# macoustics/ap-vast-unofficial

Hardware: AMD Instinct MI355X
Metric: subband filter-updates/sec (blocks x bins / s), 16-spk/32-mic/1024-bin (higher is better)
Workload: dtype f64

## Files before the change

ap_vast_unofficial_amd/csrc/gevd16_common.h:

```cpp
#pragma once
#include <type_traits>
#include "apv_internal.h"

namespace {

constexpr int N = 16;
constexpr int LD = 17;

template <typename T> struct Cx { T x, y; };
template <typename T> __device__ __forceinline__ Cx<T> mk(T a, T b) { Cx<T> r; r.x = a; r.y = b; return r; }

template <typename T> struct Prec;
template <> struct Prec<double> {
    static constexpr double sweep_tol2 = 1e-16;
    static constexpr int max_sweeps = 14;
};
template <> struct Prec<float> {
    static constexpr float sweep_tol2 = 1e-8f;
    static constexpr int max_sweeps = 12;
};

__device__ __forceinline__ double rsq_full(double x) {
    double y = __builtin_amdgcn_rsq(x);
    const double t = x * y;
    const double e = __builtin_fma(-t, y, 1.0);
    const double pp = __builtin_fma(0.375, e, 0.5);
    const double ye = y * e;
    return __builtin_fma(ye, pp, y);
}
__device__ __forceinline__ double rcp_full(double x) {
    double y = __builtin_amdgcn_rcp(x);
    y = y * __builtin_fma(-x, y, 2.0);
    return y * __builtin_fma(-x, y, 2.0);
}
__device__ __forceinline__ float rcp_full(float x) {
    const float y = __builtin_amdgcn_rcpf(x);
    return y * __builtin_fmaf(-x, y, 2.0f);
}
__device__ __forceinline__ float rsq_full(float x) {
    float y = __builtin_amdgcn_rsqf(x);
    const float t = x * y;
    const float e = __builtin_fmaf(-t, y, 1.0f);
    return __builtin_fmaf(y * e, 0.5f, y);
}

__device__ __forceinline__ void wsync() { __syncthreads(); }

template <typename T> __device__ __forceinline__ T wave_sum(T v) {
#pragma unroll
    for (int o = 32; o >= 1; o >>= 1) v += __shfl_xor(v, o, 64);
    return __shfl(v, 0, 64);
}

__device__ __forceinline__ float uniform_scalar(float v) { return __int_as_float(__builtin_amdgcn_readfirstlane(__float_as_int(v))); }
__device__ __forceinline__ double uniform_scalar(double v) {
    return __hiloint2double(__builtin_amdgcn_readfirstlane(__double2hiint(v)), __builtin_amdgcn_readfirstlane(__double2loint(v)));
}

using d4 = __attribute__((ext_vector_type(4))) double;
using f4 = __attribute__((ext_vector_type(4))) float;

template <typename T> struct Mfma16;
__device__ __forceinline__ float fma_t(float a, float b, float c) { return __builtin_fmaf(a, b, c); }
__device__ __forceinline__ double fma_t(double a, double b, double c) { return __builtin_fma(a, b, c); }

template <> struct Mfma16<double> {
    using V = d4;
    static __device__ __forceinline__ V mac(double a, double b, V c) { return __builtin_amdgcn_mfma_f64_16x16x4f64(a, b, c, 0, 0, 0); }
    static __device__ __forceinline__ int row(int lane, int t) { return (lane >> 4) + 4 * t; }
};
template <> struct Mfma16<float> {
    using V = f4;
    static __device__ __forceinline__ V mac(float a, float b, V c) { return __builtin_amdgcn_mfma_f32_16x16x4f32(a, b, c, 0, 0, 0); }
    static __device__ __forceinline__ int row(int lane, int t) { return 4 * (lane >> 4) + t; }
};

struct NoStamp { __device__ __forceinline__ void operator()(int) const {} };
template <typename T, typename XT, bool WITH_D, typename ST = NoStamp, int GS = 1>
__device__ __forceinline__ void correlate16(const XT* __restrict__ X, const XT* __restrict__ dvec, int M,
                                            Cx<T>* dst, Cx<T>* sr, int lane, ST stamp = ST(), int stamp_base = 0) {
    using MM = Mfma16<T>;
    typename MM::V re = {0, 0, 0, 0}, im = {0, 0, 0, 0};
    T rx = 0, ry = 0;
    const int msub = lane >> 4;
    XT zero;
    zero.x = 0;
    zero.y = 0;
    auto chunk = [&](int mc, auto full_tag) {
        constexpr bool FULL = decltype(full_tag)::value;
        XT xv[8], dv[8];
        const XT* const xrow0 = X + ((size_t)(mc + msub) * N + (lane & 15)) * GS;
        const XT* const drow0 = WITH_D ? dvec + mc + msub : nullptr;
#pragma unroll
        for (int q = 0; q < 8; ++q) {
            const int m = mc + 4 * q + msub;
            const bool ok = FULL || m < M;
            XT xl, dl = zero;
            if constexpr (FULL) {
                xl = xrow0[(size_t)(4 * q) * N * GS];
                if constexpr (WITH_D) dl = drow0[4 * q];
            } else {
                const int mcl = ok ? m : M - 1;
                xl = X[((size_t)mcl * N + (lane & 15)) * GS];
                if constexpr (WITH_D) dl = dvec[mcl];
            }
            xv[q].x = ok ? xl.x : zero.x;
            xv[q].y = ok ? xl.y : zero.y;
            dv[q].x = ok ? dl.x : zero.x;
            dv[q].y = ok ? dl.y : zero.y;
        }
        if constexpr (!__is_same(ST, NoStamp)) {
            asm volatile("s_waitcnt vmcnt(0)" ::: "memory");
            stamp(stamp_base);
        }
#pragma unroll
        for (int q = 0; q < 8; ++q) {
            const T xr = (T)xv[q].x, xi = (T)xv[q].y;
            re = MM::mac(xr, xr, re);
            re = MM::mac(xi, xi, re);
            im = MM::mac(xr, xi, im);
            if constexpr (WITH_D) {
                rx = fma_t(xi, (T)dv[q].y, fma_t(xr, (T)dv[q].x, rx));
                ry = fma_t(-xi, (T)dv[q].x, fma_t(xr, (T)dv[q].y, ry));
            }
        }
    };
    if ((M & 31) == 0) {
        for (int mc = 0; mc < M; mc += 32) chunk(mc, std::true_type{});
    } else {
        for (int mc = 0; mc < M; mc += 32) chunk(mc, std::false_type{});
    }
    const int col = lane & 15;
#pragma unroll
    for (int t = 0; t < 4; ++t) dst[MM::row(lane, t) * LD + col] = mk<T>(re[t], im[t]);
    stamp(stamp_base + 1);
    wsync();
    T pt[4];
#pragma unroll
    for (int t = 0; t < 4; ++t) pt[t] = dst[col * LD + MM::row(lane, t)].y;
    wsync();
#pragma unroll
    for (int t = 0; t < 4; ++t) dst[MM::row(lane, t) * LD + col].y = im[t] - pt[t];
    if constexpr (WITH_D) {
        rx += __shfl_xor(rx, 16, 64); ry += __shfl_xor(ry, 16, 64);
        rx += __shfl_xor(rx, 32, 64); ry += __shfl_xor(ry, 32, 64);
        if (lane < N) sr[lane] = mk<T>(rx, ry);
    }
}



struct XStep { signed char tbit, delta; };
constexpr XStep XSCHED[2][15] = {
    {{-1, 1}, {-1, 2}, {-1, 1}, {-1, 4}, {-1, 1}, {-1, 2}, {-1, 1}, {-1, 4}, {2, 1}, {-1, 2}, {-1, 1}, {-1, 2}, {1, 1}, {-1, 1}, {0, 0}},
    {{-1, 1}, {-1, 2}, {-1, 1}, {-1, 4}, {-1, 1}, {-1, 2}, {-1, 1}, {-1, 4}, {0, 2}, {-1, 4}, {-1, 2}, {-1, 4}, {1, 4}, {-1, 4}, {2, 0}}};
constexpr unsigned long long xs_pack(int sweep, bool tb) {
    unsigned long long v = 0;
    for (int r = 0; r < 15; ++r)
        v |= (unsigned long long)(tb ? (XSCHED[sweep][r].tbit + 1) : XSCHED[sweep][r].delta) << (4 * r);
    return v;
}
constexpr unsigned long long XS_DELTA0 = xs_pack(0, false), XS_DELTA1 = xs_pack(1, false);
constexpr unsigned long long XS_TBIT0 = xs_pack(0, true), XS_TBIT1 = xs_pack(1, true);

template <typename T> __device__ __forceinline__ Cx<T> cshfl(Cx<T> v, int src) {
    return mk<T>(__shfl(v.x, src, 64), __shfl(v.y, src, 64));
}
template <typename T> __device__ __forceinline__ void xchg(Cx<T>& top, Cx<T>& bot, bool bit, int peer) {
    const Cx<T> send = bit ? top : bot;
    const Cx<T> recv = cshfl(send, peer);
    if (bit) top = recv; else bot = recv;
}

template <int D> __device__ __forceinline__ int dpp_xor_lo(int v);
template <> __device__ __forceinline__ int dpp_xor_lo<1>(int v) { return __builtin_amdgcn_mov_dpp(v, 0xB1, 0xf, 0xf, false); }
template <> __device__ __forceinline__ int dpp_xor_lo<2>(int v) { return __builtin_amdgcn_mov_dpp(v, 0x4E, 0xf, 0xf, false); }
template <> __device__ __forceinline__ int dpp_xor_lo<4>(int v) { return __builtin_amdgcn_ds_swizzle(v, 0x101F); }
__device__ __forceinline__ int dpp_xor8(int v) { return __builtin_amdgcn_mov_dpp(v, 0x128, 0xf, 0xf, false); }

template <int D> __device__ __forceinline__ float xcol(float v) { return __int_as_float(dpp_xor_lo<D>(__float_as_int(v))); }
template <int D> __device__ __forceinline__ double xcol(double v) {
    return __hiloint2double(dpp_xor_lo<D>(__double2hiint(v)), dpp_xor_lo<D>(__double2loint(v)));
}
template <int D> __device__ __forceinline__ float xrow(float v, int lane) {
    if constexpr (D == 1) return __int_as_float(dpp_xor8(__float_as_int(v)));
    else return __int_as_float(__builtin_amdgcn_ds_bpermute((lane ^ (8 * D)) << 2, __float_as_int(v)));
}
template <int D> __device__ __forceinline__ double xrow(double v, int lane) {
    if constexpr (D == 1) return __hiloint2double(dpp_xor8(__double2hiint(v)), dpp_xor8(__double2loint(v)));
    else {
        const int addr = (lane ^ (8 * D)) << 2;
        return __hiloint2double(__builtin_amdgcn_ds_bpermute(addr, __double2hiint(v)),
                                __builtin_amdgcn_ds_bpermute(addr, __double2loint(v)));
    }
}
template <int TB> __device__ __forceinline__ void xswap_row(int& top, int& bot) {
    if constexpr (TB == 0) {
        const int nt = __builtin_amdgcn_update_dpp(top, bot, 0x128, 0xf, 0xc, false);
        bot = __builtin_amdgcn_update_dpp(bot, top, 0x128, 0xf, 0x3, false);
        top = nt;
    } else if constexpr (TB == 1) {
        const auto r = __builtin_amdgcn_permlane16_swap((unsigned)top, (unsigned)bot, false, false);
        top = (int)r[0];
        bot = (int)r[1];
    } else {
        const auto r = __builtin_amdgcn_permlane32_swap((unsigned)top, (unsigned)bot, false, false);
        top = (int)r[0];
        bot = (int)r[1];
    }
}
__device__ __forceinline__ void xswap_col4(int& top, int& bot) {
    const int nt = __builtin_amdgcn_update_dpp(top, bot, 0x114, 0xf, 0xa, false);
    bot = __builtin_amdgcn_update_dpp(bot, top, 0x104, 0xf, 0x5, false);
    top = nt;
}
template <int TB> __device__ __forceinline__ void xswap_row(float& t, float& b) {
    int ti = __float_as_int(t), bi = __float_as_int(b);
    xswap_row<TB>(ti, bi);
    t = __int_as_float(ti);
    b = __int_as_float(bi);
}
template <int TB> __device__ __forceinline__ void xswap_row(double& t, double& b) {
    int tl = __double2loint(t), th = __double2hiint(t), bl = __double2loint(b), bh = __double2hiint(b);
    xswap_row<TB>(tl, bl);
    xswap_row<TB>(th, bh);
    t = __hiloint2double(th, tl);
    b = __hiloint2double(bh, bl);
}
__device__ __forceinline__ void xswap_col4(float& t, float& b) {
    int ti = __float_as_int(t), bi = __float_as_int(b);
    xswap_col4(ti, bi);
    t = __int_as_float(ti);
    b = __int_as_float(bi);
}
__device__ __forceinline__ void xswap_col4(double& t, double& b) {
    int tl = __double2loint(t), th = __double2hiint(t), bl = __double2loint(b), bh = __double2hiint(b);
    xswap_col4(tl, bl);
    xswap_col4(th, bh);
    t = __hiloint2double(th, tl);
    b = __hiloint2double(bh, bl);
}
template <int TB, typename T> __device__ __forceinline__ void cxswap_row(Cx<T>& t, Cx<T>& b) {
    xswap_row<TB>(t.x, b.x);
    xswap_row<TB>(t.y, b.y);
}
template <typename T> __device__ __forceinline__ void cxswap_col4(Cx<T>& t, Cx<T>& b) {
    xswap_col4(t.x, b.x);
    xswap_col4(t.y, b.y);
}

template <int D, typename T> __device__ __forceinline__ Cx<T> cxcol(Cx<T> v) { return mk<T>(xcol<D>(v.x), xcol<D>(v.y)); }
template <int D, typename T> __device__ __forceinline__ Cx<T> cxrow(Cx<T> v, int lane) { return mk<T>(xrow<D>(v.x, lane), xrow<D>(v.y, lane)); }

template <int D, typename T>
__device__ __forceinline__ void move_bottoms(Cx<T>& tb, Cx<T>& bt, Cx<T>& bb, Cx<T>& v0b, Cx<T>& v1b, int lane) {
    tb = cxcol<D>(tb);
    v0b = cxcol<D>(v0b);
    v1b = cxcol<D>(v1b);
    bb = cxcol<D>(bb);
    bt = cxrow<D>(bt, lane);
    bb = cxrow<D>(bb, lane);
}

template <typename T>
__device__ __forceinline__ void rot_cols(T c, Cx<T> s, Cx<T> p, Cx<T> q, Cx<T>& po, Cx<T>& qo) {
    po.x = c * p.x - (s.x * q.x + s.y * q.y);
    po.y = c * p.y - (s.x * q.y - s.y * q.x);
    qo.x = c * q.x + (s.x * p.x - s.y * p.y);
    qo.y = c * q.y + (s.x * p.y + s.y * p.x);
}
template <typename T>
__device__ __forceinline__ void rot_rows(T c, Cx<T> s, Cx<T> p, Cx<T> q, Cx<T>& po, Cx<T>& qo) {
    po.x = c * p.x - (s.x * q.x - s.y * q.y);
    po.y = c * p.y - (s.x * q.y + s.y * q.x);
    qo.x = c * q.x + (s.x * p.x + s.y * p.y);
    qo.y = c * q.y + (s.x * p.y - s.y * p.x);
}
using f2v = __attribute__((ext_vector_type(2))) float;
using f4v = __attribute__((ext_vector_type(4))) float;
__device__ __forceinline__ f2v pk_cmul(f2v s, f2v z) {
    const f2v t = {-s.y, s.y};
    return __builtin_elementwise_fma((f2v){s.x, s.x}, z, t * (f2v){z.y, z.x});
}
__device__ __forceinline__ f2v pk_cmulc(f2v s, f2v z) {
    const f2v t = {s.y, -s.y};
    return __builtin_elementwise_fma((f2v){s.x, s.x}, z, t * (f2v){z.y, z.x});
}
template <>
__device__ __forceinline__ void rot_cols<float>(float c, Cx<float> s, Cx<float> p, Cx<float> q, Cx<float>& po, Cx<float>& qo) {
    const f2v cc = {c, c}, sv = {s.x, s.y}, pv = {p.x, p.y}, qv = {q.x, q.y};
    const f2v a = cc * pv - pk_cmulc(sv, qv), b = cc * qv + pk_cmul(sv, pv);
    po = mk<float>(a.x, a.y);
    qo = mk<float>(b.x, b.y);
}
template <>
__device__ __forceinline__ void rot_rows<float>(float c, Cx<float> s, Cx<float> p, Cx<float> q, Cx<float>& po, Cx<float>& qo) {
    const f2v cc = {c, c}, sv = {s.x, s.y}, pv = {p.x, p.y}, qv = {q.x, q.y};
    const f2v a = cc * pv - pk_cmul(sv, qv), b = cc * qv + pk_cmulc(sv, pv);
    po = mk<float>(a.x, a.y);
    qo = mk<float>(b.x, b.y);
}

template <typename T>
__device__ __forceinline__ void rotation(T alpha, T gamma, T bx, T by, T& c, T& sx, T& sy) {
    const float fbx = (float)bx, fby = (float)by, fd = (float)(gamma - alpha);
    const float b2 = fbx * fbx + fby * fby;
    if constexpr (sizeof(T) == 4) {
        const float zeta = 0.5f * fd;
        const float x = fmaxf(__builtin_fmaf(zeta, zeta, b2), 1e-36f);
        const float hh = x * __builtin_amdgcn_rsqf(x);
        const float D = fmaxf(fabsf(zeta), 1e-18f) + hh;
        const float rr = __builtin_amdgcn_rsqf((hh + hh) * D);
        const float rs = copysignf(rr, zeta);
        c = D * rr;
        sx = fbx * rs;
        sy = fby * rs;
        return;
    }
    float tx = 0.f, ty = 0.f;
    if (b2 > 1e-30f) {
        const float iab = __builtin_amdgcn_rsqf(b2);
        const float tau = fd * 0.5f * iab;
        const float rho = __builtin_amdgcn_sqrtf(__builtin_fmaf(tau, tau, 1.0f));
        const float t = copysignf(__builtin_amdgcn_rcpf(fabsf(tau) + rho), tau) * iab;
        tx = fbx * t;
        ty = fby * t;
    }
    const T dx = (T)tx, dy = (T)ty;
    c = rsq_full((T)1 + dx * dx + dy * dy);
    sx = dx * c;
    sy = dy * c;
}

template <typename TT>
__device__ __forceinline__ int jacobi16_sweeps(Cx<TT>& tt_, Cx<TT>& tb_, Cx<TT>& bt_, Cx<TT>& bb_, Cx<TT>& v0t_, Cx<TT>& v0b_,
                                               Cx<TT>& v1t_, Cx<TT>& v1b_, TT (*srot)[4], int lane, TT tol2, TT normS2,
                                               int max_sweeps, bool& converged_, int n_rounds = 15) {
    using CC = Cx<TT>;
    const int a = lane >> 3, b = lane & 7;
    const bool diag = (a == b);
    int sweeps_done = 0;
    bool converged = false;
    CC tt = tt_, tb = tb_, bt = bt_, bb = bb_, v0t = v0t_, v0b = v0b_, v1t = v1t_, v1b = v1b_;
    for (int sweep = 0; sweep < max_sweeps && !converged; ++sweep) {
        TT off = 0;
        const unsigned long long dseq = (sweep & 1) ? XS_DELTA1 : XS_DELTA0;
        const unsigned long long tseq = (sweep & 1) ? XS_TBIT1 : XS_TBIT0;
        for (int r = 0; r < n_rounds; ++r) {
            const int delta = (int)((dseq >> (4 * r)) & 15), tbit = (int)((tseq >> (4 * r)) & 15) - 1;
            if (tbit >= 0) {
                if (tbit == 2) {
                    cxswap_col4(tt, tb);
                    cxswap_col4(bt, bb);
                    cxswap_col4(v0t, v0b);
                    cxswap_col4(v1t, v1b);
                    cxswap_row<2>(tt, bt);
                    cxswap_row<2>(tb, bb);
                } else {
                    const bool cb_ = (b >> tbit) & 1;
                    const int pc = lane ^ (1 << tbit);
                    xchg(tt, tb, cb_, pc);
                    xchg(bt, bb, cb_, pc);
                    xchg(v0t, v0b, cb_, pc);
                    xchg(v1t, v1b, cb_, pc);
                    if (tbit == 1) {
                        cxswap_row<1>(tt, bt);
                        cxswap_row<1>(tb, bb);
                    } else {
                        cxswap_row<0>(tt, bt);
                        cxswap_row<0>(tb, bb);
                    }
                }
            }
            switch (delta) {
                case 1: move_bottoms<1>(tb, bt, bb, v0b, v1b, lane); break;
                case 2: move_bottoms<2>(tb, bt, bb, v0b, v1b, lane); break;
                case 4: move_bottoms<4>(tb, bt, bb, v0b, v1b, lane); break;
                default: break;
            }
            if (diag) off += tb.x * tb.x + tb.y * tb.y;
            TT c, sx, sy;
            rotation<TT>(tt.x, bb.x, tb.x, tb.y, c, sx, sy);
            TT ca, sax, say, cb, sbx, sby;
            if constexpr (sizeof(TT) == 8) {
                if (diag) {
                    srot[a][0] = c;
                    srot[a][1] = sx;
                    srot[a][2] = sy;
                }
                wsync();
                ca = srot[a][0]; sax = srot[a][1]; say = srot[a][2];
                cb = srot[b][0]; sbx = srot[b][1]; sby = srot[b][2];
            } else {
                const int da = 9 * a, db = 9 * b;
                ca = __shfl(c, da, 64); sax = __shfl(sx, da, 64); say = __shfl(sy, da, 64);
                cb = __shfl(c, db, 64); sbx = __shfl(sx, db, 64); sby = __shfl(sy, db, 64);
            }
            const CC sa = mk<TT>(sax, say), sb = mk<TT>(sbx, sby);
            CC ypp, ypq, yqp, yqq;
            rot_cols<TT>(cb, sb, tt, tb, ypp, ypq);
            rot_cols<TT>(cb, sb, bt, bb, yqp, yqq);
            rot_rows<TT>(ca, sa, ypp, yqp, tt, bt);
            rot_rows<TT>(ca, sa, ypq, yqq, tb, bb);
            if (diag) {
                tt.y = 0;
                bb.y = 0;
            }
            CC w0p, w0q, w1p, w1q;
            rot_cols<TT>(cb, sb, v0t, v0b, w0p, w0q);
            rot_cols<TT>(cb, sb, v1t, v1b, w1p, w1q);
            v0t = w0p; v0b = w0q; v1t = w1p; v1b = w1q;
        }
// ... 316 lines not shown
```

ap_vast_unofficial_amd/csrc/kernels_gevd16m.hip:

```cpp
#include "apv_internal.h"

#include <cstdlib>

#include "gevd16_common.h"

namespace {

__device__ __forceinline__ float tp_lane(float v, int l) { return __int_as_float(__builtin_amdgcn_readlane(__float_as_int(v), l)); }
__device__ __forceinline__ float tp_from(float v, int src) { return __int_as_float(__builtin_amdgcn_ds_bpermute(src << 2, __float_as_int(v))); }
__device__ __forceinline__ float tp_quad_bcast(float v, int j) {
    const int x = __float_as_int(v);
    return __int_as_float(j == 0 ? __builtin_amdgcn_mov_dpp(x, 0x00, 0xf, 0xf, false) : j == 1 ? __builtin_amdgcn_mov_dpp(x, 0x55, 0xf, 0xf, false)
                          : j == 2 ? __builtin_amdgcn_mov_dpp(x, 0xAA, 0xf, 0xf, false) : __builtin_amdgcn_mov_dpp(x, 0xFF, 0xf, 0xf, false));
}
template <int CTRL> __device__ __forceinline__ void tp_dpp_add(float& v) {
    v += __int_as_float(__builtin_amdgcn_update_dpp(0, __float_as_int(v), CTRL, 0xf, 0xf, true));
    asm volatile("" : "+v"(v));
}
__device__ __forceinline__ float tp_sum_quad(float v) { tp_dpp_add<0xB1>(v); tp_dpp_add<0x4E>(v); return v; }
__device__ __forceinline__ float tp_sum_quads(float v) {
    tp_dpp_add<0x128>(v);
    tp_dpp_add<0x124>(v);
    asm("s_nop 1\n\tv_add_f32_dpp %0, %0, %0 row_bcast:15 row_mask:0xa bank_mask:0xf\n\t"
        "s_nop 1\n\tv_add_f32_dpp %0, %0, %0 row_bcast:31 row_mask:0xc bank_mask:0xf" : "+v"(v));
// ... 337 lines not shown
        }
        const T inv2 = rcp_full(dkk);
        const C li2 = mk<T>(li.x * inv2, li.y * inv2);
#pragma unroll
        for (int t = 0; t < 4; ++t) {
            if (4 * t + 3 <= kk) continue;
            brow[t].x = fma_t(-li2.y, lj[t].y, fma_t(-li2.x, lj[t].x, brow[t].x));
            brow[t].y = fma_t(li2.x, lj[t].y, fma_t(-li2.y, lj[t].x, brow[t].y));
        }
        if (i > kk) {
#pragma unroll
            for (int t = 0; t < 4; ++t) {
                if (4 * t > kk) continue;
                wrow[t].x = fma_t(li2.y, wk[t].y, fma_t(-li2.x, wk[t].x, wrow[t].x));
                wrow[t].y = fma_t(-li2.y, wk[t].x, fma_t(-li2.x, wk[t].y, wrow[t].y));
            }
        }
    }
    wsync();
    {
        const T di = ccol[i][i].x;
        if (__any(!(di > (T)0) || !(di < (T)3.0e38))) status = 1;
        if (status == 0) {
            const T ri = rsq_full(di);
#pragma unroll
            for (int t = 0; t < 4; ++t) wrow[t] = mk<T>(wrow[t].x * ri, wrow[t].y * ri);
        }
    }
    stamp(2);
    if (dstop == 2) return;

    if (status == 0) {
#pragma unroll
        for (int t = 0; t < 4; ++t) sB[i * LD + jq + 4 * t] = wrow[t];
        wsync();
        C acc[4];
        const int col = lane & 15;
        cmm16([&](int r, int kx) { return sB[r * LD + kx]; }, [&](int kx, int c) { return sA[kx * LD + c]; }, lane, acc);
        wsync();
#pragma unroll
        for (int t = 0; t < 4; ++t) sA[mfma_row<T>(lane, t) * LD + col] = acc[t];
        wsync();
        cmm16([&](int r, int kx) { return sA[r * LD + kx]; },
              [&](int kx, int c) { const C w = sB[c * LD + kx]; return mk<T>(w.x, -w.y); }, lane, acc);
        wsync();
        T nrm = 0;
#pragma unroll
        for (int t = 0; t < 4; ++t) {
            const int row = mfma_row<T>(lane, t);
            if (row == col) acc[t].y = 0;
            sA[row * LD + col] = acc[t];
            nrm += acc[t].x * acc[t].x + acc[t].y * acc[t].y;
        }
        const T normF2 = uniform_scalar(wave_sum(nrm));
        wsync();
        stamp(3);
        if (dstop == 3) return;

        const int a = lane >> 3, b = lane & 7;
        const int max_sweeps = p.max_sweeps > 0 ? p.max_sweeps : Prec<T>::max_sweeps;
        const T tol2 = p.sweep_tol2 > 0.0 ? (T)p.sweep_tol2 : Prec<T>::sweep_tol2;
        bool converged = false;
        const int sexp = __builtin_amdgcn_readfirstlane((normF2 > (T)0) ? -((sizeof(T) == 8 ? ilogb((double)normF2) : ilogbf((float)normF2)) / 2) : 0);
        T normS2;
        if constexpr (sizeof(T) == 8) normS2 = uniform_scalar((T)ldexp((double)normF2, 2 * sexp));
        else normS2 = uniform_scalar((T)ldexpf((float)normF2, 2 * sexp));
        bool v_in_lds = false, refined = false;
        auto spectrum_ok = [&](float nt, float nb) {
            float mn = fminf(nt, nb), mx = fmaxf(nt, nb);
#pragma unroll
            for (int m = 1; m < 64; m <<= 1) {
                mn = fminf(mn, __shfl_xor(mn, m, 64));
                mx = fmaxf(mx, __shfl_xor(mx, m, 64));
            }
            return !__any(!(mn >= 1e-3f * mx));
        };
        if constexpr (sizeof(T) == 8) {
            if (dstop != 4) {
                using CF = Cx<float>;
                CF v32[4];
                CF* const fQ = reinterpret_cast<CF*>(&sB[0]);
                const bool trust = tridiag_presolve16<T>(sA, sexp, (float)normS2, fQ, reinterpret_cast<float*>(fQ + N * LDQ), lane, v32, stamp);
                if (!trust) {
                    wsync();
#pragma unroll
                    for (int t = 0; t < 4; ++t) sB[i * LD + jq + 4 * t] = wrow[t];
                    wsync();
                } else {
                const int mcol = lane & 15;
                auto cj = [](C w) { return mk<T>(w.x, -w.y); };
                wsync();
#pragma unroll
                for (int t = 0; t < 4; ++t) sB[mfma_row<float>(lane, t) * LD + mcol] = mk<T>((T)v32[t].x, (T)v32[t].y);
                wsync();
                C accT[4], accG[4], accC[4], accV[4];
                cmm16([&](int r, int kx) { return sA[r * LD + kx]; }, [&](int kx, int c) { return sB[kx * LD + c]; }, lane, accT);
                cmm16([&](int r, int kx) { return cj(sB[kx * LD + r]); }, [&](int kx, int c) { return sB[kx * LD + c]; }, lane, accG);
                wsync();
#pragma unroll
                for (int t = 0; t < 4; ++t) sA[mfma_row<T>(lane, t) * LD + mcol] = accT[t];
                wsync();
                cmm16([&](int r, int kx) { return cj(sB[kx * LD + r]); }, [&](int kx, int c) { return sA[kx * LD + c]; }, lane, accC);
                constexpr double kRefineGuard2 = 9e-10;
                constexpr double kSecondStep2 = 1e-4;
                const bool refine_ok = (dstop != 5) && !(p.sweep_tol2 > 0.0);
                T* const sLam2 = reinterpret_cast<T*>(&scoef[0]);
                for (int step = 0; step < 2; ++step) {
                    {
                        T num = (T)0, gd = (T)1;
                        bool has_diag = false;
#pragma unroll
                        for (int t = 0; t < 4; ++t) {
                            const bool d = mfma_row<T>(lane, t) == mcol;
                            num = d ? accC[t].x : num;
                            gd = d ? accG[t].x : gd;
                            has_diag = has_diag || d;
                        }
                        T ginv = __builtin_amdgcn_rcp(gd);
                        ginv = ginv * __builtin_fma(-gd, ginv, (T)2);
                        T quot = num * ginv;
                        quot = __builtin_fma(__builtin_fma(-gd, quot, num), ginv, quot);
                        if (has_diag) sLam[mcol] = quot;
                    }
                    wsync();
                    bool bad = false, hopeless = false;
                    const T dj = sLam[mcol];
                    T l2 = (T)0;
#pragma unroll
                    for (int t = 0; t < 4; ++t) {
                        const int row = mfma_row<T>(lane, t);
                        const T di = sLam[row];
                        C z;
                        if (row == mcol) {
                            z = mk<T>((T)0.5 * ((T)1 - accG[t].x), (T)0);
                        } else {
                            const T den = dj - di;
                            T inv = __builtin_amdgcn_rcp(den);
                            inv = inv * __builtin_fma(-den, inv, (T)2);
                            const T zx = __builtin_fma(-dj, accG[t].x, accC[t].x) * inv, zy = __builtin_fma(-dj, accG[t].y, accC[t].y) * inv;
                            const T zz = zx * zx + zy * zy;
                            bad = bad || !(zz <= (T)kRefineGuard2);
                            hopeless = hopeless || !(zz <= (T)kSecondStep2);
                            z = mk<T>(zx, zy);
                            l2 = __builtin_fma(zz, den, l2);
                        }
                        sA[row * LD + mcol] = z;
                    }
                    l2 += __shfl_xor(l2, 16, 64);
                    l2 += __shfl_xor(l2, 32, 64);
                    if (lane < N) sLam2[mcol] = l2 + dj;
                    const bool pass = !__any(bad) || dstop == 10;
                    if (dstop == 9 && !pass) status = 8 << step;
                    if (!refine_ok || (!pass && (step == 1 || __any(hopeless)))) break;
                    wsync();
                    auto v_step = [&]() {
                        cmm16([&](int r, int kx) { return sB[r * LD + kx]; }, [&](int kx, int c) { return sA[kx * LD + c]; }, lane, accV);
#pragma unroll
                        for (int t = 0; t < 4; ++t) {
                            const C v = sB[mfma_row<T>(lane, t) * LD + mcol];
                            accV[t] = mk<T>(v.x + accV[t].x, v.y + accV[t].y);
                        }
                    };
                    if (pass) {
                        v_step();
                        if (lane < N) sLam[lane] = sLam2[lane];
                        wsync();
#pragma unroll
                        for (int t = 0; t < 4; ++t) {
                            sA[mfma_row<T>(lane, t) * LD + mcol] = accV[t];
                            sB[i * LD + jq + 4 * t] = wrow[t];
                        }
                        wsync();
                        refined = true;
                        break;
                    }
                    if constexpr (sizeof(T) == 8) {
                        auto ipz = [&](int r, int c) { const C zv = sA[r * LD + c]; return mk<T>(zv.x + (r == c ? (T)1 : (T)0), zv.y); };
                        cmm16x([&](int s_, int, int) { return cj(accC[s_]); }, [&](int, int kx, int c) { return ipz(kx, c); }, lane, accT);
                        cmm16x([&](int, int r, int kx) { return cj(ipz(kx, r)); }, [&](int s_, int, int) { return accT[s_]; }, lane, accC);
#pragma unroll
                        for (int t = 0; t < 4; ++t)
                            if (mfma_row<T>(lane, t) == mcol) accC[t].y = 0;
                        v_step();
                        wsync();
#pragma unroll
                        for (int t = 0; t < 4; ++t) sB[mfma_row<T>(lane, t) * LD + mcol] = accV[t];
                        wsync();
                        cmm16([&](int r, int kx) { return cj(sB[kx * LD + r]); }, [&](int kx, int c) { return sB[kx * LD + c]; }, lane, accG);
                    }
                }
                if (!refined) {
                    constexpr int n_it = 4;
                    {
                    for (int it = 0; it < n_it; ++it) {
                        wsync();
#pragma unroll
                        for (int t = 0; t < 4; ++t) {
                            const int row = mfma_row<T>(lane, t);
                            sA[row * LD + mcol] = mk<T>((row == mcol ? (T)1.5 : (T)0) - (T)0.5 * accG[t].x, (T)-0.5 * accG[t].y);
                        }
                        wsync();
                        cmm16([&](int r, int kx) { return sB[r * LD + kx]; }, [&](int kx, int c) { return sA[kx * LD + c]; }, lane, accV);
                        cmm16x([&](int s_, int, int) { return cj(accC[s_]); }, [&](int, int kx, int c) { return sA[kx * LD + c]; }, lane, accT);
                        cmm16x([&](int, int r, int kx) { return sA[r * LD + kx]; }, [&](int s_, int, int) { return accT[s_]; }, lane, accC);
                        wsync();
#pragma unroll
                        for (int t = 0; t < 4; ++t) {
                            sB[mfma_row<T>(lane, t) * LD + mcol] = accV[t];
                            if (mfma_row<T>(lane, t) == mcol) accC[t].y = 0;
                        }
                        wsync();
                        if (it + 1 < n_it)
                            cmm16([&](int r, int kx) { return cj(sB[kx * LD + r]); }, [&](int kx, int c) { return sB[kx * LD + c]; }, lane, accG);
                    }
#pragma unroll
                    for (int t = 0; t < 4; ++t) sA[mfma_row<T>(lane, t) * LD + mcol] = accC[t];
                    wsync();
                    }
                    v_in_lds = true;
                }
                }
            }
        }
        if constexpr (sizeof(T) == 4) {
            constexpr int LDF = 17;
            constexpr float kShift = 8e-6f;
            const float delta = kShift * sqrtf((float)normS2);
            Cx<float>* const fG = reinterpret_cast<Cx<float>*>(&sB[0]);
            Cx<float> (*const fcol)[16] = reinterpret_cast<Cx<float>(*)[16]>(&scol[0][0]);
            chol16_f32<T, LD, LDF>(sA, sexp, delta, fG, fcol, lane);
            const int oa = lane & 7, ob = lane >> 3;
            Cx<float> g0t = fG[(2 * oa) * LDF + ob], g0b = fG[(2 * oa) * LDF + 8 + ob];
            Cx<float> g1t = fG[(2 * oa + 1) * LDF + ob], g1b = fG[(2 * oa + 1) * LDF + 8 + ob];
            float n2t, n2b;
            (void)jacobi16_onesided<LDF>(g0t, g0b, g1t, g1b, lane, (float)tol2, (float)normS2, max_sweeps, converged, n2t, n2b, fG);
            const bool trust = converged && spectrum_ok(n2t, n2b);
            converged = false;
            wsync();
#pragma unroll
            for (int t = 0; t < 4; ++t) sB[i * LD + jq + 4 * t] = wrow[t];
            if (trust) {
                const int it_b = os_top_end(ob), ib_b = os_bot_end(ob);
                wsync();
                sA[(2 * oa) * LD + it_b] = mk<T>(g0t.x, g0t.y);
                sA[(2 * oa) * LD + ib_b] = mk<T>(g0b.x, g0b.y);
                sA[(2 * oa + 1) * LD + it_b] = mk<T>(g1t.x, g1t.y);
                sA[(2 * oa + 1) * LD + ib_b] = mk<T>(g1b.x, g1b.y);
                if (oa == 0) {
                    sLam[it_b] = (T)ldexpf(n2t - delta, -sexp);
                    sLam[ib_b] = (T)ldexpf(n2b - delta, -sexp);
                }
                refined = true;
            }
            wsync();
        }
        if (!refined) {
            C tt = sA[a * LD + b], tb = sA[a * LD + 8 + b], bt = sA[(8 + a) * LD + b], bb = sA[(8 + a) * LD + 8 + b];
            const T scl = (sizeof(T) == 8) ? (T)ldexp(1.0, sexp) : (T)ldexpf(1.0f, sexp);
            tt = mk<T>(tt.x * scl, tt.y * scl); tb = mk<T>(tb.x * scl, tb.y * scl);
            bt = mk<T>(bt.x * scl, bt.y * scl); bb = mk<T>(bb.x * scl, bb.y * scl);
            C v0t = mk<T>((2 * a == b) ? (T)1 : (T)0, 0), v0b = mk<T>((2 * a == 8 + b) ? (T)1 : (T)0, 0);
            C v1t = mk<T>((2 * a + 1 == b) ? (T)1 : (T)0, 0), v1b = mk<T>((2 * a + 1 == 8 + b) ? (T)1 : (T)0, 0);
            if (v_in_lds) {
                v0t = sB[(2 * a) * LD + b]; v0b = sB[(2 * a) * LD + 8 + b];
                v1t = sB[(2 * a + 1) * LD + b]; v1b = sB[(2 * a + 1) * LD + 8 + b];
                wsync();
    #pragma unroll
                for (int t = 0; t < 4; ++t) sB[i * LD + jq + 4 * t] = wrow[t];
            }
            const bool diag = (a == b);
            const int sweeps_done = jacobi16_sweeps<T>(tt, tb, bt, bb, v0t, v0b, v1t, v1b, srot, lane, tol2, normS2, max_sweeps, converged);
            if (!converged) status = 2;
            const bool nat = sweeps_done & 1;
            const int it_b = nat ? 2 * b : b, ib_b = nat ? 2 * b + 1 : 8 + b;
            wsync();
            sA[(2 * a) * LD + it_b] = v0t;
            sA[(2 * a) * LD + ib_b] = v0b;
            sA[(2 * a + 1) * LD + it_b] = v1t;
            sA[(2 * a + 1) * LD + ib_b] = v1b;
            if (diag) {
                const T iscl = (sizeof(T) == 8) ? (T)ldexp(1.0, -sexp) : (T)ldexpf(1.0f, -sexp);
                sLam[it_b] = tt.x * iscl;
                sLam[ib_b] = bb.x * iscl;
            }
            wsync();
        }

        stamp(6);
        {
            const int i16 = lane & 15, q4 = lane >> 4;
            const T li = sLam[i16];
            int rank = 0;
#pragma unroll
            for (int jj = 0; jj < 4; ++jj) {
                const int j = 4 * q4 + jj;
                const T lj = sLam[j];
                rank += (lj > li) || (lj == li && j < i16);
            }
            rank += __shfl_xor(rank, 16, 64);
            rank += __shfl_xor(rank, 32, 64);
            if (q4 == 0) sOrder[rank] = i16;
        }

        cmm16([&](int r, int kx) { const C w = sB[kx * LD + r]; return mk<T>(w.x, -w.y); },
              [&](int kx, int c) { return sA[kx * LD + c]; }, lane, acc);
        wsync();
#pragma unroll
        for (int t = 0; t < 4; ++t) sA[mfma_row<T>(lane, t) * LD + col] = acc[t];
        wsync();

        {
            const int i16 = lane & 15, q4 = lane >> 4;
            T sx = 0, sy = 0;
#pragma unroll
            for (int ll = 0; ll < 4; ++ll) {
                const int l = 4 * q4 + ll;
                const C v = sA[l * LD + i16], rr = sr[l];
                sx = fma_t(v.y, rr.y, fma_t(v.x, rr.x, sx));
                sy = fma_t(-v.y, rr.x, fma_t(v.x, rr.y, sy));
            }
            sx += __shfl_xor(sx, 16, 64); sy += __shfl_xor(sy, 16, 64);
            sx += __shfl_xor(sx, 32, 64); sy += __shfl_xor(sy, 32, 64);
            if (q4 == 0) {
                const T den = rcp_full(sLam[i16] + span_mu<true, T>(p.span, z1, k, p.mu));
                scoef[i16] = mk<T>(sx * den, sy * den);
            }
        }
        wsync();
    }

    {
        const int i16 = lane & 15;
        T ax = 0, ay = 0;
        int done = lane >> 4;
        const int s_k = span_limit<true, T>(p.span, z1, k, N, p.ranks[p.nV - 1], status != 1, !HOPS || hop == p.span.last_hop, sLam,
                                      scoef, sOrder, lane);
        for (int t = 0; t < p.nV; ++t) {
            const int V = min(p.ranks[t], s_k);
            if (status != 1) {
                for (; done < V; done += 4) {
                    const int c = sOrder[done];
                    const C cf = scoef[c], v = sA[i16 * LD + c];
                    ax = fma_t(-cf.y, v.y, fma_t(cf.x, v.x, ax));
                    ay = fma_t(cf.y, v.x, fma_t(cf.x, v.y, ay));
                }
            }
            T wx = ax + __shfl_xor(ax, 16, 64), wy = ay + __shfl_xor(ay, 16, 64);
            wx += __shfl_xor(wx, 32, 64); wy += __shfl_xor(wy, 32, 64);
            if (lane < N) {
                const size_t o = ((size_t)k * p.nV + t) * N + lane;
                if (p.out_c128) reinterpret_cast<double2*>(pw)[o] = make_double2((double)wx, (double)wy);
                else reinterpret_cast<float2*>(pw)[o] = make_float2((float)wx, (float)wy);
            }
        }
    }
    if (lane < N) {
        if (plam != nullptr) {
            const T lv = (status != 1) ? sLam[sOrder[lane]] : (T)0;
            if (p.out_c128) reinterpret_cast<double*>(plam)[(size_t)k * N + lane] = (double)lv;
            else reinterpret_cast<float*>(plam)[(size_t)k * N + lane] = (float)lv;
        }
    }
    if (p.U != nullptr) {
        C* U = reinterpret_cast<C*>(p.U) + (size_t)k * N * N;
#pragma unroll
        for (int t = 0; t < 4; ++t) {
            const int idx = lane + 64 * t, ii = idx >> 4, j = idx & 15;
            U[idx] = (status != 1) ? sA[ii * LD + sOrder[j]] : mk<T>(0, 0);
        }
    }
    if (pstatus != nullptr && lane == 0) pstatus[k] = status;
    stamp(7);
}

template <typename T, bool FUSED, typename XT, bool DBG = false>
__global__ void __launch_bounds__(64) gevd16m_kernel(const GevdParams p) { gevd16m_body<T, FUSED, XT, DBG>(p, blockIdx.x, blockIdx.y == 1); }
template <bool FUSED, typename XT, bool DBG = false>
__global__ void __launch_bounds__(64) __attribute__((amdgpu_waves_per_eu(4, 4))) gevd16m_kernel_f64(const GevdParams p) {
    gevd16m_body<double, FUSED, XT, DBG>(p, blockIdx.x, blockIdx.y == 1);
}
template <int GS>
__global__ void __launch_bounds__(64) __attribute__((amdgpu_waves_per_eu(4, 4))) gevd16m_kernel_f64_grouped(const GevdParams p) {
    constexpr int BLK = 8 * GS;
    const int id = blockIdx.x;
    const int k = ((id | (BLK - 1)) < p.K) ? ((id & ~(BLK - 1)) | ((id & 7) * GS) | ((id >> 3) & (GS - 1))) : id;
    gevd16m_body<double, true, double2, false, GS>(p, k, blockIdx.y == 1);
}
template <int GS>
__global__ void __launch_bounds__(64) __attribute__((amdgpu_waves_per_eu(4, 4))) gevd16m_kernel_f64_hops(const GevdParams p) {
    constexpr int BLK = 8 * GS;
    const int id = blockIdx.x;
    const int k = (GS > 1 && (id | (BLK - 1)) < p.K) ? ((id & ~(BLK - 1)) | ((id & 7) * GS) | ((id >> 3) & (GS - 1))) : id;
    gevd16m_body<double, true, double2, false, GS, true>(p, k, blockIdx.y == 1, blockIdx.z);
}

__global__ void __launch_bounds__(64) __attribute__((amdgpu_waves_per_eu(4, 4))) gevd16m_kernel_f64_hops_c64(const GevdParams p) {
    gevd16m_body<double, true, float2, false, 1, true>(p, blockIdx.x, blockIdx.y == 1, blockIdx.z);
}
__global__ void __launch_bounds__(64) gevd16m_kernel_f32_hops_c64(const GevdParams p) {
    gevd16m_body<float, true, float2, false, 1, true>(p, blockIdx.x, blockIdx.y == 1, blockIdx.z);
}

}

bool apv_gevd16m_takes_hops(const GevdParams& p, int compute_dtype, bool fused) {
    if (!(p.n == 16 && p.reg_mode == APV_REG_ABS && p.reg_bright == 0.0 && fused && p.debug_stop == 0 && p.stamps == nullptr && p.n_hops <= 65535))
        return false;
    if (p.x_c128) return compute_dtype == APV_F64 && (p.x_group <= 1 || p.x_group == 4);
    return p.x_group <= 1;
}

hipError_t apv_launch_gevd16m(const GevdParams& p, int compute_dtype, bool fused, hipStream_t s) {
    if (p.n != 16 || p.reg_mode != APV_REG_ABS || p.reg_bright != 0.0) return hipErrorNotSupported;
    if (p.K <= 0) return hipSuccess;
    const dim3 grid(p.K, p.n_zones > 1 ? 2 : 1);
    const bool xd = fused && p.x_c128;
    if (p.n_hops > 1) {
        if (!apv_gevd16m_takes_hops(p, compute_dtype, fused)) return hipErrorInvalidValue;
        const dim3 grid3(p.K, p.n_zones > 1 ? 2 : 1, p.n_hops);
        if (!p.x_c128) {
            if (compute_dtype == APV_F64) hipLaunchKernelGGL(gevd16m_kernel_f64_hops_c64, grid3, dim3(64), 0, s, p);
            else hipLaunchKernelGGL(gevd16m_kernel_f32_hops_c64, grid3, dim3(64), 0, s, p);
            return hipGetLastError();
        }
        if (p.x_group == 4) hipLaunchKernelGGL(gevd16m_kernel_f64_hops<4>, grid3, dim3(64), 0, s, p);
        else hipLaunchKernelGGL(gevd16m_kernel_f64_hops<1>, grid3, dim3(64), 0, s, p);
        return hipGetLastError();
    }
    if (p.x_group > 1) {
        if (!xd || compute_dtype != APV_F64 || p.debug_stop != 0 || p.stamps != nullptr) return hipErrorInvalidValue;
        if (p.x_group == 4) hipLaunchKernelGGL(gevd16m_kernel_f64_grouped<4>, grid, dim3(64), 0, s, p);
        else return hipErrorInvalidValue;
        return hipGetLastError();
    }
    if (p.debug_stop != 0 || p.stamps != nullptr) {
        if (compute_dtype == APV_F64) {
            if (xd) hipLaunchKernelGGL((gevd16m_kernel_f64<true, double2, true>), grid, dim3(64), 0, s, p);
            else if (fused) hipLaunchKernelGGL((gevd16m_kernel_f64<true, float2, true>), grid, dim3(64), 0, s, p);
            else hipLaunchKernelGGL((gevd16m_kernel_f64<false, float2, true>), grid, dim3(64), 0, s, p);
        } else {
            if (xd) hipLaunchKernelGGL((gevd16m_kernel<float, true, double2, true>), grid, dim3(64), 0, s, p);
            else if (fused) hipLaunchKernelGGL((gevd16m_kernel<float, true, float2, true>), grid, dim3(64), 0, s, p);
            else hipLaunchKernelGGL((gevd16m_kernel<float, false, float2, true>), grid, dim3(64), 0, s, p);
        }
        return hipGetLastError();
    }
    if (compute_dtype == APV_F64) {
        if (xd) hipLaunchKernelGGL((gevd16m_kernel_f64<true, double2>), grid, dim3(64), 0, s, p);
        else if (fused) hipLaunchKernelGGL((gevd16m_kernel_f64<true, float2>), grid, dim3(64), 0, s, p);
        else hipLaunchKernelGGL((gevd16m_kernel_f64<false, float2>), grid, dim3(64), 0, s, p);
    } else {
        if (xd) hipLaunchKernelGGL((gevd16m_kernel<float, true, double2>), grid, dim3(64), 0, s, p);
        else if (fused) hipLaunchKernelGGL((gevd16m_kernel<float, true, float2>), grid, dim3(64), 0, s, p);
        else hipLaunchKernelGGL((gevd16m_kernel<float, false, float2>), grid, dim3(64), 0, s, p);
    }
    return hipGetLastError();
}
```

Before: 102.5 million.

## Replace full back-transform matmul with matrix-vector products in GEVD filter path

Instead of forming the full 16x16 back-transformed eigenvector matrix with an MFMA matmul every bin, the kernel now applies B^H to the cross-correlation vector (a mat-vec) and then maps the weighted eigenvector sum back through B with another mat-vec per output rank. The full matmul is kept only when U is requested. The correlate loop also defers its masking of out-of-range samples until after all loads are issued, so the loads can overlap. The cost is extra syncs and shuffles per rank in the output loop.

Measured after the change: 103.8 million, median of 6. 1.01x the previous value.

```diff
diff --git a/ap_vast_unofficial_amd/csrc/gevd16_common.h b/ap_vast_unofficial_amd/csrc/gevd16_common.h
--- a/ap_vast_unofficial_amd/csrc/gevd16_common.h
+++ b/ap_vast_unofficial_amd/csrc/gevd16_common.h
@@ -93,21 +93,30 @@
         const XT* const drow0 = WITH_D ? dvec + mc + msub : nullptr;
 #pragma unroll
         for (int q = 0; q < 8; ++q) {
-            const int m = mc + 4 * q + msub;
-            const bool ok = FULL || m < M;
             XT xl, dl = zero;
             if constexpr (FULL) {
                 xl = xrow0[(size_t)(4 * q) * N * GS];
                 if constexpr (WITH_D) dl = drow0[4 * q];
             } else {
-                const int mcl = ok ? m : M - 1;
+                const int m = mc + 4 * q + msub;
+                const int mcl = m < M ? m : M - 1;
                 xl = X[((size_t)mcl * N + (lane & 15)) * GS];
                 if constexpr (WITH_D) dl = dvec[mcl];
             }
-            xv[q].x = ok ? xl.x : zero.x;
-            xv[q].y = ok ? xl.y : zero.y;
-            dv[q].x = ok ? dl.x : zero.x;
-            dv[q].y = ok ? dl.y : zero.y;
+            xv[q] = xl;
+            dv[q] = dl;
+        }
+        if constexpr (!FULL) {
+#pragma unroll
+            for (int q = 0; q < 8; ++q) {
+                asm volatile("" : "+v"(xv[q].x), "+v"(xv[q].y));
+                if constexpr (WITH_D) asm volatile("" : "+v"(dv[q].x), "+v"(dv[q].y));
+                const bool ok = mc + 4 * q + msub < M;
+                xv[q].x = ok ? xv[q].x : zero.x;
+                xv[q].y = ok ? xv[q].y : zero.y;
+                dv[q].x = ok ? dv[q].x : zero.x;
+                dv[q].y = ok ? dv[q].y : zero.y;
+            }
         }
         if constexpr (!__is_same(ST, NoStamp)) {
             asm volatile("s_waitcnt vmcnt(0)" ::: "memory");
diff --git a/ap_vast_unofficial_amd/csrc/kernels_gevd16m.hip b/ap_vast_unofficial_amd/csrc/kernels_gevd16m.hip
--- a/ap_vast_unofficial_amd/csrc/kernels_gevd16m.hip
+++ b/ap_vast_unofficial_amd/csrc/kernels_gevd16m.hip
@@ -663,11 +663,21 @@
             if (q4 == 0) sOrder[rank] = i16;
         }
 
-        cmm16([&](int r, int kx) { const C w = sB[kx * LD + r]; return mk<T>(w.x, -w.y); },
-              [&](int kx, int c) { return sA[kx * LD + c]; }, lane, acc);
-        wsync();
-#pragma unroll
-        for (int t = 0; t < 4; ++t) sA[mfma_row<T>(lane, t) * LD + col] = acc[t];
+        {
+            const int i16 = lane & 15, q4 = lane >> 4;
+            T gx = 0, gy = 0;
+#pragma unroll
+            for (int ll = 0; ll < 4; ++ll) {
+                const int l = 4 * q4 + ll;
+                const C w = sB[i16 * LD + l], rr = sr[l];
+                gx = fma_t(-w.y, rr.y, fma_t(w.x, rr.x, gx));
+                gy = fma_t(w.y, rr.x, fma_t(w.x, rr.y, gy));
+            }
+            gx += __shfl_xor(gx, 16, 64); gy += __shfl_xor(gy, 16, 64);
+            gx += __shfl_xor(gx, 32, 64); gy += __shfl_xor(gy, 32, 64);
+            wsync();
+            if (q4 == 0) sr[i16] = mk<T>(gx, gy);
+        }
         wsync();
 
         {
@@ -691,9 +701,12 @@
     }
 
     {
-        const int i16 = lane & 15;
+        const int i16 = lane & 15, q4 = lane >> 4;
         T ax = 0, ay = 0;
-        int done = lane >> 4;
+        int done = q4;
+        C wl[4];
+#pragma unroll
+        for (int ll = 0; ll < 4; ++ll) wl[ll] = (status != 1) ? sB[(4 * q4 + ll) * LD + i16] : mk<T>(0, 0);
         const int s_k = span_limit<true, T>(p.span, z1, k, N, p.ranks[p.nV - 1], status != 1, !HOPS || hop == p.span.last_hop, sLam,
                                       scoef, sOrder, lane);
         for (int t = 0; t < p.nV; ++t) {
@@ -706,7 +719,19 @@
                     ay = fma_t(cf.y, v.x, fma_t(cf.x, v.y, ay));
                 }
             }
-            T wx = ax + __shfl_xor(ax, 16, 64), wy = ay + __shfl_xor(ay, 16, 64);
+            T yx = ax + __shfl_xor(ax, 16, 64), yy = ay + __shfl_xor(ay, 16, 64);
+            yx += __shfl_xor(yx, 32, 64); yy += __shfl_xor(yy, 32, 64);
+            wsync();
+            if (q4 == 0) sr[i16] = mk<T>(yx, yy);
+            wsync();
+            T wx = 0, wy = 0;
+#pragma unroll
+            for (int ll = 0; ll < 4; ++ll) {
+                const C y = sr[4 * q4 + ll];
+                wx = fma_t(wl[ll].y, y.y, fma_t(wl[ll].x, y.x, wx));
+                wy = fma_t(-wl[ll].y, y.x, fma_t(wl[ll].x, y.y, wy));
+            }
+            wx += __shfl_xor(wx, 16, 64); wy += __shfl_xor(wy, 16, 64);
             wx += __shfl_xor(wx, 32, 64); wy += __shfl_xor(wy, 32, 64);
             if (lane < N) {
                 const size_t o = ((size_t)k * p.nV + t) * N + lane;
@@ -723,6 +748,15 @@
         }
     }
     if (p.U != nullptr) {
+        if (status != 1) {
+            C xacc[4];
+            cmm16([&](int r, int kx) { const C w = sB[kx * LD + r]; return mk<T>(w.x, -w.y); },
+                  [&](int kx, int c) { return sA[kx * LD + c]; }, lane, xacc);
+            wsync();
+#pragma unroll
+            for (int t = 0; t < 4; ++t) sA[mfma_row<T>(lane, t) * LD + (lane & 15)] = xacc[t];
+            wsync();
+        }
         C* U = reinterpret_cast<C*>(p.U) + (size_t)k * N * N;
 #pragma unroll
         for (int t = 0; t < 4; ++t) {
```
